# ppwwyyxx/speaker-recognition

Measured on AMD Instinct MI355X. Metric: frames/sec scored (MFCC+GMM), higher is better.
Workload: dtype f32

## Files before the change

speaker-recognition_amd/csrc/mfcc_f64.hip:

```cpp
#include "batch.hpp"
#include "mfcc.hpp"
#include "mfcc_dev.hpp"
#include "wave_ops.hpp"

#include <algorithm>

namespace sr {

static int &precision_flag() {
    static int v = 2;
    return v;
}
int mfcc_precision() { return precision_flag(); }
void mfcc_set_precision(int mode) { precision_flag() = mode == 0 ? 0 : 2; }

using d2 = double2;

__device__ __forceinline__ d2 mk(double x, double y) { return make_double2(x, y); }
__device__ __forceinline__ d2 dadd(d2 a, d2 b) { return mk(a.x + b.x, a.y + b.y); }
__device__ __forceinline__ d2 dsub(d2 a, d2 b) { return mk(a.x - b.x, a.y - b.y); }
__device__ __forceinline__ d2 dmul(d2 a, d2 b) { return mk(fma(-a.y, b.y, a.x * b.x), fma(a.y, b.x, a.x * b.y)); }
__device__ __forceinline__ d2 dmul_mi(d2 a) { return mk(a.y, -a.x); }
constexpr double DH = 0.70710678118654752440;
__device__ __forceinline__ d2 dmul_h_mh(d2 a) { return mk(DH * (a.x + a.y), DH * (a.y - a.x)); }
__device__ __forceinline__ d2 dmul_mh_mh(d2 a) { return mk(DH * (a.y - a.x), -DH * (a.x + a.y)); }

__device__ __forceinline__ d2 tw64(const d2 *t, int i, int nc) {
    d2 w = t[i & (nc - 1)];
    if (i & nc) w = mk(-w.x, -w.y);
    return w;
}

__device__ __forceinline__ void radix4d(d2 a, d2 b, d2 c, d2 d, d2 &y0, d2 &y1, d2 &y2, d2 &y3) {
    const d2 s0 = dadd(a, c), s1 = dsub(a, c), s2 = dadd(b, d), s3 = dmul_mi(dsub(b, d));
    y0 = dadd(s0, s2);
    y1 = dadd(s1, s3);
    y2 = dsub(s0, s2);
    y3 = dsub(s1, s3);
}

template <int NZ>
__device__ __forceinline__ void dft16d(d2 (&v)[16]) {
    constexpr double C1 = 0.92387953251128673848, S1 = 0.38268343236508978178;
    d2 u[4][4];
    if constexpr (NZ <= 4) {
#pragma unroll
        for (int q = 0; q < 4; q++)
#pragma unroll
            for (int r = 0; r < 4; r++) u[q][r] = v[q];
    } else {
#pragma unroll
        for (int q = 0; q < 4; q++) radix4d(v[q], v[4 + q], v[8 + q], v[12 + q], u[q][0], u[q][1], u[q][2], u[q][3]);
    }
    u[1][1] = dmul(u[1][1], mk(C1, -S1));
    u[1][2] = dmul_h_mh(u[1][2]);
    u[1][3] = dmul(u[1][3], mk(S1, -C1));
    u[2][1] = dmul_h_mh(u[2][1]);
    u[2][2] = dmul_mi(u[2][2]);
    u[2][3] = dmul_mh_mh(u[2][3]);
    u[3][1] = dmul(u[3][1], mk(S1, -C1));
    u[3][2] = dmul_mh_mh(u[3][2]);
    u[3][3] = dmul(u[3][3], mk(-C1, S1));
#pragma unroll
    for (int r = 0; r < 4; r++) radix4d(u[0][r], u[1][r], u[2][r], u[3][r], v[r], v[r + 4], v[r + 8], v[r + 12]);
}

template <int CTRL>
__device__ __forceinline__ float quad_f32(float x) {
    return __int_as_float(__builtin_amdgcn_update_dpp(0, __float_as_int(x), CTRL, 0xf, 0xf, true));
}
template <int CTRL>
__device__ __forceinline__ double quad_f64(double x) {
    union { double d; int i[2]; } a, b;
    a.d = x;
    b.i[0] = __builtin_amdgcn_update_dpp(0, a.i[0], CTRL, 0xf, 0xf, true);
    b.i[1] = __builtin_amdgcn_update_dpp(0, a.i[1], CTRL, 0xf, 0xf, true);
    return b.d;
}
constexpr int QUAD_XOR1 = 0xB1;
constexpr int QUAD_XOR2 = 0x4E;

__device__ constexpr double W32_COS[9] = {1.0, 0.98078528040323044913, 0.92387953251128675613, 0.83146961230254523708,
                                          0.70710678118654752440, 0.55557023301960222474, 0.38268343236508977173,
                                          0.19509032201612826785, 0.0};

__device__ __forceinline__ double ln_pos_f32(float e) {
    int ex;
    float m = frexpf(e, &ex);
    if (m < 0.70710678f) {
        m *= 2.0f;
        ex -= 1;
    }
    const double md = (double)m, den = md + 1.0;
    double r = (double)__builtin_amdgcn_rcpf((float)den);
    r = fma(r, fma(-den, r, 1.0), r);
    const double s = (md - 1.0) * r, s2 = s * s;
    double c15 = 1.0 / 15.0, c13 = 1.0 / 13.0, c11 = 1.0 / 11.0, c9 = 1.0 / 9.0, c7 = 1.0 / 7.0, c5 = 1.0 / 5.0, c3 = 1.0 / 3.0, ln2 = 0.69314718055994530942;
    asm volatile("" : "+s"(c15), "+s"(c13), "+s"(c11), "+s"(c9), "+s"(c7), "+s"(c5), "+s"(c3), "+s"(ln2));
    double p = c15;
    p = fma(p, s2, c13);
    p = fma(p, s2, c11);
    p = fma(p, s2, c9);
    p = fma(p, s2, c7);
    p = fma(p, s2, c5);
    p = fma(p, s2, c3);
    p = fma(p, s2, 1.0);
    return fma((double)ex, ln2, 2.0 * s * p);
}

constexpr int F64_U_ELEMS = 576;
constexpr int F64_PBUF_BYTE = F64_U_ELEMS * 16;
constexpr int F64_SE_BYTE = F64_PBUF_BYTE + 1100 * 4;
constexpr int F64_SLM_BYTE = F64_SE_BYTE + 272;
static_assert(F64_SLM_BYTE % 32 == 0 && F64_SLM_BYTE + 512 <= WAVE_SLAB_C * 16, "per-wave slab layout");

template <typename PcmT, int MP>
__global__ __launch_bounds__(64 * F64_WPB)
void mfcc_frames_fft2048_f64_kernel(const PcmT *__restrict__ pcm, const int64_t *__restrict__ sample_off,
                                    const int64_t *__restrict__ frame_off, int n_utt, int64_t n_frames,
                                    int64_t frames_per_wave, MfccDev p, MfccDev64 q, MelRuns mr, float *__restrict__ raw) {
    extern __shared__ __attribute__((aligned(32))) char smem[];
    constexpr int NC = 1024;
    float *s_melval = reinterpret_cast<float *>(smem);
    const int lane = threadIdx.x & 63;
    const int wave = threadIdx.x >> 6;
    double *s_win = reinterpret_cast<double *>(smem + (((size_t)mr.pad_floats * 4 + 31) & ~(size_t)31));
    char *slab_b = reinterpret_cast<char *>(s_win) + F64_WIN_BYTES + (size_t)wave * WAVE_SLAB_C * sizeof(d2);
    d2 *slab = reinterpret_cast<d2 *>(slab_b);
    float *pbuf = reinterpret_cast<float *>(slab_b + F64_PBUF_BYTE);
    float *s_e = reinterpret_cast<float *>(slab_b + F64_SE_BYTE);
    double *s_lm = reinterpret_cast<double *>(slab_b + F64_SLM_BYTE);

    for (int i = threadIdx.x; i < mr.pad_floats; i += 64 * F64_WPB) s_melval[i] = mr.pad_val[i];
    for (int i = threadIdx.x; i < F64_WIN_BYTES / 8; i += 64 * F64_WPB) s_win[i] = (i >= 1 && i <= p.frame_len) ? q.window[i - 1] : 0.0;
    __syncthreads();

    const d2 w1 = q.twiddle[2 * lane];
    const d2 wl = q.twiddle[lane];
    const int bb = lane & 15, gg = lane >> 4;
    const d2 w64_1 = q.twiddle[32 * bb];
    const int L = p.frame_len;
    const double lm_floor = q.mel_floor[lane];
    const int m_part = lane & 3, m_bl = lane >> 2;
    int m_c0[4];
#pragma unroll
    for (int ps = 0; ps < 4; ps++) m_c0[ps] = mr.col0[16 * ps + m_bl];

    const int64_t gwave = (int64_t)blockIdx.x * F64_WPB + wave;
    const int64_t f_begin = gwave * frames_per_wave;
    const int64_t f_end = f_begin + frames_per_wave < n_frames ? f_begin + frames_per_wave : n_frames;
    if (f_begin >= f_end) return;

    int utt = 0;
    {
        int lo = 0, hi = n_utt;
        while (hi - lo > 1) {
            const int mid = (lo + hi) >> 1;
            if (frame_off[mid] <= f_begin) lo = mid; else hi = mid;
        }
        utt = lo;
    }
    int64_t utt_f0 = frame_off[utt], utt_f1 = frame_off[utt + 1], utt_s0 = sample_off[utt];

    PcmT cm[4], c0[4], c1[4];
    auto fetch = [&](int64_t base) {
        const PcmT *fp = pcm + base;
#pragma unroll
        for (int n1 = 0; n1 < 4; n1++) {
            const int i0 = 2 * (64 * n1 + lane);
            c0[n1] = fp[min(i0, L - 1)];
            cm[n1] = fp[max(min(i0 - 1, L - 1), 0)];
            c1[n1] = fp[min(i0 + 1, L - 1)];
        }
    };
    fetch(utt_s0 + (f_begin - utt_f0) * p.frame_shift);

    for (int64_t frame = f_begin; frame < f_end; frame++) {
        d2 v[16];
#pragma unroll
        for (int n1 = 0; n1 < 4; n1++) {
            const int i0 = 2 * (64 * n1 + lane);
            const d2 wm0 = *reinterpret_cast<const d2 *>(s_win + i0);
            const double wp1 = s_win[i0 + 2];
            const double x0 = (double)c0[n1], xm = (double)cm[n1], x1 = (double)c1[n1];
            const double y0 = wm0.y * x0;
            const double re = fma(-(wm0.x * q.pre_emph), xm, y0);
            const double im = fma(-q.pre_emph, y0, wp1 * x1);
            v[n1] = mk(i0 < L ? re : 0.0, i0 + 1 < L ? im : 0.0);
        }
        if (frame + 1 < f_end) {
            int64_t nf = frame + 1;
            while (nf >= utt_f1) {
                utt++;
                utt_f0 = utt_f1;
                utt_f1 = frame_off[utt + 1];
                utt_s0 = sample_off[utt];
            }
            fetch(utt_s0 + (nf - utt_f0) * p.frame_shift);
        }
        dft16d<4>(v);
        {
            d2 cur = w1;
            v[1] = dmul(v[1], cur);
#pragma unroll
            for (int k1 = 2; k1 < 16; k1++) {
                cur = dmul(cur, w1);
                v[k1] = dmul(v[k1], cur);
            }
        }
        wave_sync();
#pragma unroll
        for (int k1 = 0; k1 < 16; k1++) slab[k1 * 68 + lane] = v[k1];
        wave_sync();
        {
            d2 w64_2 = dmul(w64_1, w64_1);
            asm volatile("" : "+v"(w64_2.x), "+v"(w64_2.y));
            const d2 w64_3 = dmul(w64_2, w64_1);
#pragma unroll
            for (int i = 0; i < 4; i++) {
                const d2 *rowp = slab + (4 * gg + i) * 68 + bb;
                radix4d(rowp[0], rowp[16], rowp[32], rowp[48], v[4 * i], v[4 * i + 1], v[4 * i + 2], v[4 * i + 3]);
                v[4 * i + 1] = dmul(v[4 * i + 1], w64_1);
                v[4 * i + 2] = dmul(v[4 * i + 2], w64_2);
                v[4 * i + 3] = dmul(v[4 * i + 3], w64_3);
            }
        }
        wave_sync();
#pragma unroll
        for (int i = 0; i < 4; i++)
#pragma unroll
            for (int c = 0; c < 4; c++) slab[((4 * gg + i) + 16 * c) * 17 + bb] = v[4 * i + c];
        wave_sync();
#pragma unroll
        for (int b = 0; b < 16; b++) v[b] = slab[lane * 17 + b];
        dft16d<16>(v);
        wave_sync();
#pragma unroll
        for (int d = 8; d < 16; d++) slab[(d - 8) * 64 + lane] = v[d];
        wave_sync();
        {
            const int src = (64 - lane) & 63;
            const int shift = lane == 0 ? 64 : 0;
#pragma unroll
            for (int d = 0; d < 8; d++) {
                const d2 zk = v[d];
                d2 zr = slab[(7 - d) * 64 + shift + src];
                if (d == 0 && lane == 0) zr = zk;
                const d2 e = mk(zk.x + zr.x, zk.y - zr.y);
                const d2 o = mk(zk.y + zr.y, zr.x - zk.x);
                d2 t;
                if (d == 0) t = dmul(wl, o);
                else if (d == 4) t = dmul(wl, dmul_h_mh(o));
                else t = dmul(wl, dmul(mk(W32_COS[d], -W32_COS[8 - d]), o));
                const d2 xp = dadd(e, t), xm = dsub(e, t);
                const int k = lane + 64 * d;
                pbuf[k] = (float)fma(xp.x, xp.x, xp.y * xp.y);
                pbuf[NC - k] = (float)fma(xm.x, xm.x, xm.y * xm.y);
            }
            if (lane == 0) pbuf[512] = (float)(4.0 * fma(v[8].x, v[8].x, v[8].y * v[8].y));
            pbuf[1025 + lane] = 0.f;
            if (lane < 11) pbuf[1089 + lane] = 0.f;
        }
        double dw[4][4];
        int dct_lane = lane;
        asm volatile("" : "+v"(dct_lane));
#pragma unroll
        for (int it = 0; it < 4; it++) {
            const double4 wv = reinterpret_cast<const double4 *>(q.dct_pad)[it * 64 + dct_lane];
            dw[it][0] = wv.x; dw[it][1] = wv.y; dw[it][2] = wv.z; dw[it][3] = wv.w;
        }
        wave_sync();
#pragma unroll
        for (int ps = 0; ps < 4; ps++) {
            const int len = mr.pass_len[ps];
            const float4 *mv4 = reinterpret_cast<const float4 *>(s_melval + mr.pass_base[ps]) + lane;
            int c0v = m_c0[ps];
            if constexpr (MP == 0) {
                int bl = 16 * ps + m_bl;
                asm volatile("" : "+v"(bl));
                c0v = mr.col0[bl];
            }
            const float4 *pp4 = reinterpret_cast<const float4 *>(pbuf + c0v) + m_part;
            float a0 = 0.f, a1 = 0.f, a2 = 0.f, a3 = 0.f;
            if constexpr (MP != 0) {
#pragma unroll
                for (int it = 0; it < mel_preset_steps(MP, ps); it++) {
                    const float4 wv = mv4[it * 64];
                    const float4 xv = pp4[it * 4];
                    a0 = fmaf(wv.x, xv.x, a0);
                    a1 = fmaf(wv.y, xv.y, a1);
                    a2 = fmaf(wv.z, xv.z, a2);
                    a3 = fmaf(wv.w, xv.w, a3);
                }
            } else {
                for (int it = 0; it < (len >> 4); it++) {
                    const float4 wv = mv4[it * 64];
                    const float4 xv = pp4[it * 4];
                    a0 = fmaf(wv.x, xv.x, a0);
                    a1 = fmaf(wv.y, xv.y, a1);
                    a2 = fmaf(wv.z, xv.z, a2);
                    a3 = fmaf(wv.w, xv.w, a3);
                }
            }
            float acc = (a0 + a1) + (a2 + a3);
            acc += quad_f32<QUAD_XOR1>(acc);
            acc += quad_f32<QUAD_XOR2>(acc);
            if (m_part == 0) s_e[16 * ps + m_bl] = acc;
        }
        wave_sync();
        {
            const float e = s_e[lane];
            s_lm[lane] = e > 0.f ? ln_pos_f32(e) : lm_floor;
        }
        wave_sync();
        {
            const int cidx = lane >> 2;
            const double4 *lp = reinterpret_cast<const double4 *>(s_lm) + m_part;
            double o0 = 0.0, o1 = 0.0;
#pragma unroll
            for (int it = 0; it < 4; it++) {
                const double4 lv = lp[it * 4];
                o0 = fma(dw[it][0], lv.x, o0);
                o1 = fma(dw[it][1], lv.y, o1);
                o0 = fma(dw[it][2], lv.z, o0);
                o1 = fma(dw[it][3], lv.w, o1);
            }
            double o = o0 + o1;
            o += quad_f64<QUAD_XOR1>(o);
            o += quad_f64<QUAD_XOR2>(o);
            if (m_part == 0 && cidx < p.n_ceps) raw[frame * p.n_ceps + cidx] = (float)o;
        }
    }
}

template <typename PcmT, int WPB>
__global__ __launch_bounds__(64 * WPB)
void mfcc_frames_f64_kernel(const PcmT *__restrict__ pcm, const int64_t *__restrict__ sample_off,
                            const int64_t *__restrict__ frame_off, int n_utt, int64_t n_frames,
                            MfccDev p, MfccDev64 q, float *__restrict__ raw ) {
    extern __shared__ __attribute__((aligned(16))) char smem[];
    const int nc = p.fft_size >> 1;
    d2 *s_tw = reinterpret_cast<d2 *>(smem);
    const int lane = threadIdx.x & 63;
    const int wave = threadIdx.x >> 6;
    d2 *buf_a = s_tw + nc + (size_t)wave * 2 * nc;
    d2 *buf_b = buf_a + nc;
    double *s_lm = reinterpret_cast<double *>(s_tw + nc + (size_t)WPB * 2 * nc) + wave * 64;

    for (int i = threadIdx.x; i < nc; i += 64 * WPB) s_tw[i] = q.twiddle[i];
    __syncthreads();

    const int64_t frames_per_iter = (int64_t)gridDim.x * WPB;
    const int64_t iters = (n_frames + frames_per_iter - 1) / frames_per_iter;
    for (int64_t it = 0; it < iters; it++) {
        const int64_t frame = (it * gridDim.x + blockIdx.x) * WPB + wave;
        const bool active = frame < n_frames;

        int64_t base = 0;
        if (active) {
            int lo = 0, hi = n_utt;
            while (hi - lo > 1) {
                const int mid = (lo + hi) >> 1;
                if (frame_off[mid] <= frame) lo = mid; else hi = mid;
            }
            base = sample_off[lo] + (frame - frame_off[lo]) * p.frame_shift;
        }

        if (active) {
            const int L = p.frame_len;
            for (int n = lane; n < nc; n += 64) {
                double re = 0.0, im = 0.0;
                const int i0 = 2 * n;
                if (i0 < L) {
                    const double c0 = (double)pcm[base + i0] * q.window[i0];
                    const double pm1 = i0 > 0 ? (double)pcm[base + i0 - 1] * q.window[i0 - 1] : 0.0;
                    re = i0 > 0 ? c0 - pm1 * q.pre_emph : c0;
                    if (i0 + 1 < L) {
                        const double c1 = (double)pcm[base + i0 + 1] * q.window[i0 + 1];
                        im = c1 - c0 * q.pre_emph;
                    }
                }
                buf_a[n] = mk(re, im);
            }
        }
        __syncthreads();

        d2 *in = buf_a, *out = buf_b;
        int ns = 1;
        for (; ns * 4 <= nc; ns *= 4) {
            if (active) {
                const int T = nc >> 2;
                const int tstep = p.fft_size / (4 * ns);
                for (int j = lane; j < T; j += 64) {
                    const int k = j & (ns - 1);
                    const int qq = k * tstep;
                    const d2 v0 = in[j];
                    const d2 v1 = dmul(in[j + T], tw64(s_tw, qq, nc));
                    const d2 v2 = dmul(in[j + 2 * T], tw64(s_tw, 2 * qq, nc));
                    const d2 v3 = dmul(in[j + 3 * T], tw64(s_tw, 3 * qq, nc));
                    d2 y0, y1, y2, y3;
                    radix4d(v0, v1, v2, v3, y0, y1, y2, y3);
                    const int j0 = ((j - k) << 2) + k;
                    out[j0] = y0;
                    out[j0 + ns] = y1;
                    out[j0 + 2 * ns] = y2;
                    out[j0 + 3 * ns] = y3;
                }
            }
            __syncthreads();
            d2 *t = in; in = out; out = t;
        }
        if (ns < nc) {
            if (active) {
                const int T = nc >> 1;
                for (int j = lane; j < T; j += 64) {
                    const d2 v0 = in[j];
                    const d2 v1 = dmul(in[j + T], tw64(s_tw, 2 * j, nc));
                    out[j] = dadd(v0, v1);
                    out[j + T] = dsub(v0, v1);
                }
            }
            __syncthreads();
            d2 *t = in; in = out; out = t;
        }

        double *pw = reinterpret_cast<double *>(out);
        if (active) {
            for (int k = lane; k <= nc; k += 64) {
                const d2 zk = in[k & (nc - 1)];
                const d2 zr = in[(nc - k) & (nc - 1)];
                const d2 e = mk(0.5 * (zk.x + zr.x), 0.5 * (zk.y - zr.y));
                const d2 o = mk(0.5 * (zk.y + zr.y), -0.5 * (zk.x - zr.x));
                const d2 x = dadd(e, dmul(tw64(s_tw, k, nc), o));
                const double pk = fma(x.x, x.x, x.y * x.y);
                pw[k] = pk < 1e-100 ? 1e-100 : pk;
            }
        }
        __syncthreads();

        if (active) {
            double mine = 0.0;
            for (int b = 0; b < p.n_filters; b++) {
                double acc = 0.0;
                const int e1 = p.mel_row[b + 1];
                for (int e = p.mel_row[b] + lane; e < e1; e += 64) acc = fma(q.mel_val[e], pw[p.mel_col[e]], acc);
                acc = wave_sum_f64(acc);
                if (lane == b) mine = acc > 0.0 ? log(acc) : q.mel_floor[b];
            }
            s_lm[lane] = mine;
        }
        __syncthreads();

        if (active && lane < p.n_ceps) {
            double acc = 0.0;
            const double *drow = q.dct + lane * p.n_filters;
            for (int b = 0; b < p.n_filters; b++) acc = fma(drow[b], s_lm[b], acc);
            raw[frame * p.n_ceps + lane] = (float)acc;
        }
        __syncthreads();
    }
}

void mfcc_launch_f64(SRMfcc &m, const MfccPlan &plan, const MfccDev &dev, int pcm_kind, const void *pcm, const int64_t *d_pcm_off,
                     const int64_t *d_raw_off, int n_utt, int64_t n_frames, float *raw) {
    auto &tabs = device_tables(m);
    const MfccDev64 dev64 = device_tables_f64(m);
    const int grid = plan.grid;
    if (plan.kernel == MFCC_F64_FAST) {
        MelRuns mr;
        mr.col0 = tabs.mel_col0.p;
        mr.pad_val = tabs.mel_pad.p;
        mr.pad_floats = tabs.mel.pad_floats;
        for (int ps = 0; ps < 4; ps++) {
            mr.pass_base[ps] = tabs.mel.pass_base[ps];
            mr.pass_len[ps] = tabs.mel.pass_len[ps];
        }
        const size_t lds_fast = plan.lds;
        const int64_t frames_per_wave = plan.frames_per_wave;
        const int preset = plan.preset;
#define SR_LAUNCH_F64(PT, MPV)                                                                              \
    do {                                                                                                     \
        auto kern = mfcc_frames_fft2048_f64_kernel<PT, MPV>;                                                 \
        SR_HIP(hipFuncSetAttribute(reinterpret_cast<const void *>(kern), hipFuncAttributeMaxDynamicSharedMemorySize, (int)lds_fast)); \
        hipLaunchKernelGGL(kern, dim3(grid), dim3(64 * F64_WPB), lds_fast, ctx().stream, static_cast<const PT *>(pcm), d_pcm_off,      \
                           d_raw_off, n_utt, n_frames, frames_per_wave, dev, dev64, mr, raw);                \
    } while (0)
#define SR_LAUNCH_F64_P(PT)                                                                                 \
    do {                                                                                                     \
        if (preset == 1) SR_LAUNCH_F64(PT, 1); else SR_LAUNCH_F64(PT, 0); \
    } while (0)
        if (pcm_kind == SRBatch::PCM16) SR_LAUNCH_F64_P(int16_t); else SR_LAUNCH_F64_P(float);
#undef SR_LAUNCH_F64_P
#undef SR_LAUNCH_F64
        return;
    }
    if (plan.kernel != MFCC_F64_GENERIC) fail("MFCC plan names no float64 kernel");
    const int wpb = plan.wpb;
    const size_t lds = plan.lds;
#define SR_LAUNCH_G64(PT, W)                                                                                \
    do {                                                                                                     \
        auto kern = mfcc_frames_f64_kernel<PT, W>;                                                           \
        SR_HIP(hipFuncSetAttribute(reinterpret_cast<const void *>(kern), hipFuncAttributeMaxDynamicSharedMemorySize, (int)lds)); \
        hipLaunchKernelGGL(kern, dim3(grid), dim3(64 * W), lds, ctx().stream, static_cast<const PT *>(pcm), d_pcm_off, d_raw_off, \
                           n_utt, n_frames, dev, dev64, raw);                                                \
    } while (0)
#define SR_LAUNCH_G64_W(PT)                                                                                 \
    do {                                                                                                     \
        if (wpb == 4) SR_LAUNCH_G64(PT, 4); else if (wpb == 2) SR_LAUNCH_G64(PT, 2); else SR_LAUNCH_G64(PT, 1); \
    } while (0)
    if (pcm_kind == SRBatch::PCM16) SR_LAUNCH_G64_W(int16_t); else SR_LAUNCH_G64_W(float);
#undef SR_LAUNCH_G64_W
#undef SR_LAUNCH_G64
}

}
```

Baseline: 35.60 million.

## Restructure f64 FFT as 8x8x8 passes with split even/odd halves and interleaved exchanges

Replaces the 16x64 decomposition of the 1024-point complex FFT with radix-8 passes (8x8x8). Samples are split into even and odd halves whose LDS exchanges are interleaved with compute through sched_group_barrier hints, and a final radix-2 combine is added. Twiddles are precomputed per lane into registers instead of chained multiplies. The mel-energy LDS round trip is removed by keeping each lane's band in a register. The change adds register pressure and many new index maps, which are checked with constexpr static_asserts.

```diff
diff --git a/speaker-recognition_amd/csrc/mfcc_f64.hip b/speaker-recognition_amd/csrc/mfcc_f64.hip
--- a/speaker-recognition_amd/csrc/mfcc_f64.hip
+++ b/speaker-recognition_amd/csrc/mfcc_f64.hip
@@ -39,30 +39,100 @@
     y3 = dsub(s1, s3);
 }
 
-template <int NZ>
-__device__ __forceinline__ void dft16d(d2 (&v)[16]) {
-    constexpr double C1 = 0.92387953251128673848, S1 = 0.38268343236508978178;
-    d2 u[4][4];
-    if constexpr (NZ <= 4) {
-#pragma unroll
-        for (int q = 0; q < 4; q++)
-#pragma unroll
-            for (int r = 0; r < 4; r++) u[q][r] = v[q];
-    } else {
-#pragma unroll
-        for (int q = 0; q < 4; q++) radix4d(v[q], v[4 + q], v[8 + q], v[12 + q], u[q][0], u[q][1], u[q][2], u[q][3]);
-    }
-    u[1][1] = dmul(u[1][1], mk(C1, -S1));
-    u[1][2] = dmul_h_mh(u[1][2]);
-    u[1][3] = dmul(u[1][3], mk(S1, -C1));
-    u[2][1] = dmul_h_mh(u[2][1]);
-    u[2][2] = dmul_mi(u[2][2]);
-    u[2][3] = dmul_mh_mh(u[2][3]);
-    u[3][1] = dmul(u[3][1], mk(S1, -C1));
-    u[3][2] = dmul_mh_mh(u[3][2]);
-    u[3][3] = dmul(u[3][3], mk(-C1, S1));
-#pragma unroll
-    for (int r = 0; r < 4; r++) radix4d(u[0][r], u[1][r], u[2][r], u[3][r], v[r], v[r + 4], v[r + 8], v[r + 12]);
+__device__ __forceinline__ void dft8d(d2 (&v)[8]) {
+    d2 e0, e1, e2, e3, o0, o1, o2, o3;
+    radix4d(v[0], v[2], v[4], v[6], e0, e1, e2, e3);
+    radix4d(v[1], v[3], v[5], v[7], o0, o1, o2, o3);
+    o1 = dmul_h_mh(o1);
+    o2 = dmul_mi(o2);
+    o3 = dmul_mh_mh(o3);
+    v[0] = dadd(e0, o0); v[4] = dsub(e0, o0);
+    v[1] = dadd(e1, o1); v[5] = dsub(e1, o1);
+    v[2] = dadd(e2, o2); v[6] = dsub(e2, o2);
+    v[3] = dadd(e3, o3); v[7] = dsub(e3, o3);
+}
+
+constexpr int F64_HALF_SLOTS = WAVE_SLAB_C / 2;
+constexpr int F64_U_ELEMS = 576;
+__host__ __device__ constexpr int f64_p2_lane(int k1, int b) { return 8 * k1 + b; }
+__host__ __device__ constexpr int f64_p3_lane(int k1, int c) { return k1 + 8 * c; }
+__host__ __device__ constexpr int f64_ex1_slot(int k1, int l) { return 64 * k1 + (l ^ (8 * (k1 & 1))); }
+__host__ __device__ constexpr int f64_ex2_slot(int k1, int b, int c) { return 8 * f64_p3_lane(k1, c) + (f64_p3_lane(k1, c) >> 1) + b; }
+__host__ __device__ constexpr int f64_bin(int lane, int reg) { return lane + 64 * reg; }
+__host__ __device__ constexpr int f64_partner_lane(int lane) { return (64 - lane) & 63; }
+__host__ __device__ constexpr int f64_partner_reg(int lane, int d) { return lane == 0 ? 16 - d : 15 - d; }
+__host__ __device__ constexpr int f64_u_slot(int lane, int reg) { return (reg - 8) * 64 + lane; }
+
+namespace f64_map_checks {
+constexpr bool lanes_bijective() {
+    bool s2[64] = {}, s3[64] = {};
+    for (int k1 = 0; k1 < 8; k1++)
+        for (int x = 0; x < 8; x++) {
+            const int l2 = f64_p2_lane(k1, x), l3 = f64_p3_lane(k1, x);
+            if (l2 < 0 || l2 >= 64 || s2[l2] || l3 < 0 || l3 >= 64 || s3[l3]) return false;
+            s2[l2] = s3[l3] = true;
+        }
+    return true;
+}
+constexpr bool ex1_injective() {
+    bool seen[512] = {};
+    for (int k1 = 0; k1 < 8; k1++)
+        for (int l = 0; l < 64; l++) {
+            const int s = f64_ex1_slot(k1, l);
+            if (s < 0 || s >= 512 || seen[s]) return false;
+            if (s != f64_ex1_slot(k1 & 1, l) - 64 * (k1 & 1) + 64 * k1) return false;
+            const int a = l >> 3, b = l & 7;
+            if (s != ((a & 1) ? f64_ex1_slot(k1, 8 + b) - 8 : f64_ex1_slot(k1, b)) + 8 * a) return false;
+            seen[s] = true;
+        }
+    return 512 <= F64_HALF_SLOTS;
+}
+constexpr bool ex2_injective() {
+    bool seen[F64_HALF_SLOTS] = {};
+    for (int k1 = 0; k1 < 8; k1++)
+        for (int b = 0; b < 8; b++)
+            for (int c = 0; c < 8; c++) {
+                const int s = f64_ex2_slot(k1, b, c);
+                if (s < 0 || s >= F64_HALF_SLOTS || seen[s]) return false;
+                if (s != f64_ex2_slot(k1, b, 0) + 68 * c) return false;
+                if (s != f64_ex2_slot(k1, 0, c) + b) return false;
+                seen[s] = true;
+            }
+    return true;
+}
+constexpr bool bins_bijective() {
+    bool seen[1024] = {};
+    for (int lane = 0; lane < 64; lane++)
+        for (int reg = 0; reg < 16; reg++) {
+            const int k = f64_bin(lane, reg);
+            if (k < 0 || k >= 1024 || seen[k]) return false;
+            seen[k] = true;
+        }
+    for (int k1 = 0; k1 < 8; k1++)
+        for (int c = 0; c < 8; c++)
+            for (int d = 0; d < 8; d++)
+                if (f64_bin(f64_p3_lane(k1, c), d) != k1 + 8 * (c + 8 * d)) return false;
+    return true;
+}
+constexpr bool partner_is_mirror() {
+    bool seen[F64_U_ELEMS] = {};
+    for (int lane = 0; lane < 64; lane++)
+        for (int reg = 8; reg < 16; reg++) {
+            const int s = f64_u_slot(lane, reg);
+            if (s < 0 || s >= 512 || seen[s]) return false;
+            seen[s] = true;
+        }
+    for (int lane = 0; lane < 64; lane++)
+        for (int d = 0; d < 8; d++) {
+            const int k = f64_bin(lane, d), pl = f64_partner_lane(lane), pr = f64_partner_reg(lane, d);
+            if (k == 0) {
+                if (f64_u_slot(pl, pr) >= F64_U_ELEMS) return false;
+                continue;
+            }
+            if (pr < 8 || pr >= 16 || f64_bin(pl, pr) != 1024 - k) return false;
+        }
+    return f64_bin(0, 8) == 512;
+}
 }
 
 template <int CTRL>
@@ -108,11 +178,16 @@
     return fma((double)ex, ln2, 2.0 * s * p);
 }
 
-constexpr int F64_U_ELEMS = 576;
 constexpr int F64_PBUF_BYTE = F64_U_ELEMS * 16;
 constexpr int F64_SE_BYTE = F64_PBUF_BYTE + 1100 * 4;
 constexpr int F64_SLM_BYTE = F64_SE_BYTE + 272;
 static_assert(F64_SLM_BYTE % 32 == 0 && F64_SLM_BYTE + 512 <= WAVE_SLAB_C * 16, "per-wave slab layout");
+static_assert(2 * F64_HALF_SLOTS <= WAVE_SLAB_C && F64_U_ELEMS <= WAVE_SLAB_C, "the two halves' exchange regions lie inside the wave's slab");
+static_assert(f64_map_checks::lanes_bijective(), "pass-2 / pass-3 lane maps are bijections onto the wave");
+static_assert(f64_map_checks::ex1_injective(), "exchange 1: (k1, lane) -> slot is a bijection onto [0, 512)");
+static_assert(f64_map_checks::ex2_injective(), "exchange 2: (k1, b, c) -> slot is injective into the half's region");
+static_assert(f64_map_checks::bins_bijective(), "(lane, register) -> bin is a bijection onto [0, 1024)");
+static_assert(f64_map_checks::partner_is_mirror(), "partner(k) is where bin 1024 - k lives");
 
 template <typename PcmT, int MP>
 __global__ __launch_bounds__(64 * F64_WPB)
@@ -128,20 +203,18 @@
     char *slab_b = reinterpret_cast<char *>(s_win) + F64_WIN_BYTES + (size_t)wave * WAVE_SLAB_C * sizeof(d2);
     d2 *slab = reinterpret_cast<d2 *>(slab_b);
     float *pbuf = reinterpret_cast<float *>(slab_b + F64_PBUF_BYTE);
-    float *s_e = reinterpret_cast<float *>(slab_b + F64_SE_BYTE);
     double *s_lm = reinterpret_cast<double *>(slab_b + F64_SLM_BYTE);
 
     for (int i = threadIdx.x; i < mr.pad_floats; i += 64 * F64_WPB) s_melval[i] = mr.pad_val[i];
     for (int i = threadIdx.x; i < F64_WIN_BYTES / 8; i += 64 * F64_WPB) s_win[i] = (i >= 1 && i <= p.frame_len) ? q.window[i - 1] : 0.0;
     __syncthreads();
 
-    const d2 w1 = q.twiddle[2 * lane];
-    const d2 wl = q.twiddle[lane];
-    const int bb = lane & 15, gg = lane >> 4;
-    const d2 w64_1 = q.twiddle[32 * bb];
+    d2 w1 = q.twiddle[2 * lane];
+    d2 wl = q.twiddle[lane];
     const int L = p.frame_len;
-    const double lm_floor = q.mel_floor[lane];
     const int m_part = lane & 3, m_bl = lane >> 2;
+    const int my_band = 16 * m_part + m_bl;
+    double lm_floor = q.mel_floor[my_band];
     int m_c0[4];
 #pragma unroll
     for (int ps = 0; ps < 4; ps++) m_c0[ps] = mr.col0[16 * ps + m_bl];
@@ -162,31 +235,83 @@
     }
     int64_t utt_f0 = frame_off[utt], utt_f1 = frame_off[utt + 1], utt_s0 = sample_off[utt];
 
-    PcmT cm[4], c0[4], c1[4];
+    d2 tw1[8], tw2[8];
+#pragma unroll
+    for (int k = 1; k < 8; k++) {
+        tw1[k] = tw64(q.twiddle, 4 * lane * k, NC);
+        tw2[k] = tw64(q.twiddle, 32 * (lane & 7) * k, NC);
+        asm volatile("" : "+v"(tw1[k].x), "+v"(tw1[k].y), "+v"(tw2[k].x), "+v"(tw2[k].y));
+    }
+    asm volatile("" : "+v"(w1.x), "+v"(w1.y), "+v"(wl.x), "+v"(wl.y), "+v"(lm_floor));
+    const int p2_k1 = lane >> 3, p2_b = lane & 7;
+    const int ex1_w_even = f64_ex1_slot(0, lane), ex1_w_odd = f64_ex1_slot(1, lane) - 64;
+    const int ex1_r_even = f64_ex1_slot(p2_k1, p2_b), ex1_r_odd = f64_ex1_slot(p2_k1, 8 + p2_b) - 8;
+    const int ex2_w = f64_ex2_slot(p2_k1, p2_b, 0);
+    const int ex2_r = f64_ex2_slot(lane & 7, 0, lane >> 3);
+    d2 *const slab_e = slab, *const slab_o = slab + F64_HALF_SLOTS;
+
+    PcmT cs[2][5];
     auto fetch = [&](int64_t base) {
         const PcmT *fp = pcm + base;
 #pragma unroll
-        for (int n1 = 0; n1 < 4; n1++) {
-            const int i0 = 2 * (64 * n1 + lane);
-            c0[n1] = fp[min(i0, L - 1)];
-            cm[n1] = fp[max(min(i0 - 1, L - 1), 0)];
-            c1[n1] = fp[min(i0 + 1, L - 1)];
+        for (int n1 = 0; n1 < 2; n1++) {
+            const int i0 = 4 * (64 * n1 + lane);
+#pragma unroll
+            for (int j = 0; j < 5; j++) cs[n1][j] = fp[max(min(i0 + j - 1, L - 1), 0)];
         }
     };
     fetch(utt_s0 + (f_begin - utt_f0) * p.frame_shift);
 
+    auto pass1 = [&](const d2 x0, const d2 x1, d2 (&v)[8]) {
+        const d2 xa = dmul_h_mh(x1), xb = dmul_mi(x1), xc = dmul_mh_mh(x1);
+        v[0] = dadd(x0, x1);
+        v[1] = dmul(dadd(x0, xa), tw1[1]);
+        v[2] = dmul(dadd(x0, xb), tw1[2]);
+        v[3] = dmul(dadd(x0, xc), tw1[3]);
+        v[4] = dmul(dsub(x0, x1), tw1[4]);
+        v[5] = dmul(dsub(x0, xa), tw1[5]);
+        v[6] = dmul(dsub(x0, xb), tw1[6]);
+        v[7] = dmul(dsub(x0, xc), tw1[7]);
+    };
+    auto ex1_write = [&](d2 *hs, const d2 (&v)[8]) {
+#pragma unroll
+        for (int k1 = 0; k1 < 8; k1++) hs[((k1 & 1) ? ex1_w_odd : ex1_w_even) + 64 * k1] = v[k1];
+    };
+    auto ex1_read = [&](const d2 *hs, d2 (&v)[8]) {
+#pragma unroll
+        for (int a = 0; a < 8; a++) v[a] = hs[((a & 1) ? ex1_r_odd : ex1_r_even) + 8 * a];
+    };
+    auto pass2 = [&](d2 (&v)[8]) {
+        dft8d(v);
+#pragma unroll
+        for (int c = 1; c < 8; c++) v[c] = dmul(v[c], tw2[c]);
+    };
+    auto ex2_write = [&](d2 *hs, const d2 (&v)[8]) {
+#pragma unroll
+        for (int c = 0; c < 8; c++) hs[ex2_w + 68 * c] = v[c];
+    };
+    auto ex2_read = [&](const d2 *hs, d2 (&v)[8]) {
+#pragma unroll
+        for (int b = 0; b < 8; b++) v[b] = hs[ex2_r + b];
+    };
+
     for (int64_t frame = f_begin; frame < f_end; frame++) {
-        d2 v[16];
-#pragma unroll
-        for (int n1 = 0; n1 < 4; n1++) {
-            const int i0 = 2 * (64 * n1 + lane);
-            const d2 wm0 = *reinterpret_cast<const d2 *>(s_win + i0);
-            const double wp1 = s_win[i0 + 2];
-            const double x0 = (double)c0[n1], xm = (double)cm[n1], x1 = (double)c1[n1];
-            const double y0 = wm0.y * x0;
-            const double re = fma(-(wm0.x * q.pre_emph), xm, y0);
-            const double im = fma(-q.pre_emph, y0, wp1 * x1);
-            v[n1] = mk(i0 < L ? re : 0.0, i0 + 1 < L ? im : 0.0);
+        d2 xe[2], xo[2];
+#pragma unroll
+        for (int n1 = 0; n1 < 2; n1++) {
+            const int i0 = 4 * (64 * n1 + lane);
+            const d2 wa = *reinterpret_cast<const d2 *>(s_win + i0);
+            const d2 wb = *reinterpret_cast<const d2 *>(s_win + i0 + 2);
+            const double wc = s_win[i0 + 4];
+            const double xm = (double)cs[n1][0], x0 = (double)cs[n1][1], x1 = (double)cs[n1][2], x2 = (double)cs[n1][3],
+                         x3 = (double)cs[n1][4];
+            const double t0 = wa.y * x0, t1 = wb.x * x1, t2 = wb.y * x2;
+            const double y0 = fma(-(wa.x * q.pre_emph), xm, t0);
+            const double y1 = fma(-q.pre_emph, t0, t1);
+            const double y2 = fma(-q.pre_emph, t1, t2);
+            const double y3 = fma(-q.pre_emph, t2, wc * x3);
+            xe[n1] = mk(i0 < L ? y0 : 0.0, i0 + 1 < L ? y1 : 0.0);
+            xo[n1] = mk(i0 + 2 < L ? y2 : 0.0, i0 + 3 < L ? y3 : 0.0);
         }
         if (frame + 1 < f_end) {
             int64_t nf = frame + 1;
@@ -198,53 +323,79 @@
             }
             fetch(utt_s0 + (nf - utt_f0) * p.frame_shift);
         }
-        dft16d<4>(v);
+        d2 ve[8], vo[8];
+#define F64_SPREAD_EXCHANGE()                                                                  \
+    do {                                                                                       \
+        _Pragma("unroll") for (int i_ = 0; i_ < 8; i_++) {                                     \
+            __builtin_amdgcn_sched_group_barrier(0x200, 1, 0);               \
+            __builtin_amdgcn_sched_group_barrier(0x002, 3, 0);           \
+        }                                                                                      \
+        _Pragma("unroll") for (int i_ = 0; i_ < 8; i_++) {                                     \
+            __builtin_amdgcn_sched_group_barrier(0x100, 1, 0);                \
+            __builtin_amdgcn_sched_group_barrier(0x002, 2, 0);                                 \
+        }                                                                                      \
+    } while (0)
+        pass1(xe[0], xe[1], ve);
+        __builtin_amdgcn_sched_barrier(0);
+        wave_sync();
+        ex1_write(slab_e, ve);
+        wave_sync();
+        ex1_read(slab_e, ve);
+        pass1(xo[0], xo[1], vo);
+        F64_SPREAD_EXCHANGE();
+        __builtin_amdgcn_sched_barrier(0);
+        ex1_write(slab_o, vo);
+        wave_sync();
+        ex1_read(slab_o, vo);
+        pass2(ve);
+        F64_SPREAD_EXCHANGE();
+        __builtin_amdgcn_sched_barrier(0);
+        wave_sync();
+        ex2_write(slab_e, ve);
+        wave_sync();
+        ex2_read(slab_e, ve);
+        pass2(vo);
+        F64_SPREAD_EXCHANGE();
+        __builtin_amdgcn_sched_barrier(0);
+        wave_sync();
+        ex2_write(slab_o, vo);
+        wave_sync();
+        ex2_read(slab_o, vo);
+        dft8d(ve);
+        F64_SPREAD_EXCHANGE();
+        __builtin_amdgcn_sched_barrier(0);
+        dft8d(vo);
+#undef F64_SPREAD_EXCHANGE
+        wave_sync();
+        d2 z512;
+#pragma unroll
+        for (int d = 0; d < 8; d++) {
+            constexpr double C1 = 0.92387953251128673848, S1 = 0.38268343236508978178;
+            d2 t = vo[d];
+            if (d == 1) t = dmul(t, mk(C1, -S1));
+            else if (d == 2) t = dmul_h_mh(t);
+            else if (d == 3) t = dmul(t, mk(S1, -C1));
+            else if (d == 4) t = dmul_mi(t);
+            else if (d == 5) t = dmul(t, mk(-S1, -C1));
+            else if (d == 6) t = dmul_mh_mh(t);
+            else if (d == 7) t = dmul(t, mk(-C1, -S1));
+            t = dmul(w1, t);
+            const d2 hi = dsub(ve[d], t);
+            ve[d] = dadd(ve[d], t);
+            slab[f64_u_slot(lane, d + 8)] = hi;
+            if (d == 0) z512 = hi;
+        }
+        wave_sync();
         {
-            d2 cur = w1;
-            v[1] = dmul(v[1], cur);
-#pragma unroll
-            for (int k1 = 2; k1 < 16; k1++) {
-                cur = dmul(cur, w1);
-                v[k1] = dmul(v[k1], cur);
-            }
-        }
-        wave_sync();
-#pragma unroll
-        for (int k1 = 0; k1 < 16; k1++) slab[k1 * 68 + lane] = v[k1];
-        wave_sync();
-        {
-            d2 w64_2 = dmul(w64_1, w64_1);
-            asm volatile("" : "+v"(w64_2.x), "+v"(w64_2.y));
-            const d2 w64_3 = dmul(w64_2, w64_1);
-#pragma unroll
-            for (int i = 0; i < 4; i++) {
-                const d2 *rowp = slab + (4 * gg + i) * 68 + bb;
-                radix4d(rowp[0], rowp[16], rowp[32], rowp[48], v[4 * i], v[4 * i + 1], v[4 * i + 2], v[4 * i + 3]);
-                v[4 * i + 1] = dmul(v[4 * i + 1], w64_1);
-                v[4 * i + 2] = dmul(v[4 * i + 2], w64_2);
-                v[4 * i + 3] = dmul(v[4 * i + 3], w64_3);
-            }
-        }
-        wave_sync();
-#pragma unroll
-        for (int i = 0; i < 4; i++)
-#pragma unroll
-            for (int c = 0; c < 4; c++) slab[((4 * gg + i) + 16 * c) * 17 + bb] = v[4 * i + c];
-        wave_sync();
-#pragma unroll
-        for (int b = 0; b < 16; b++) v[b] = slab[lane * 17 + b];
-        dft16d<16>(v);
-        wave_sync();
-#pragma unroll
-        for (int d = 8; d < 16; d++) slab[(d - 8) * 64 + lane] = v[d];
-        wave_sync();
-        {
-            const int src = (64 - lane) & 63;
-            const int shift = lane == 0 ? 64 : 0;
+            const int src = f64_partner_lane(lane);
+            d2 zp[8];
+#pragma unroll
+            for (int d = 0; d < 8; d++) zp[d] = slab[f64_u_slot(src, f64_partner_reg(lane, d))];
+            __builtin_amdgcn_sched_barrier(0);
 #pragma unroll
             for (int d = 0; d < 8; d++) {
-                const d2 zk = v[d];
-                d2 zr = slab[(7 - d) * 64 + shift + src];
+                const d2 zk = ve[d];
+                d2 zr = zp[d];
                 if (d == 0 && lane == 0) zr = zk;
                 const d2 e = mk(zk.x + zr.x, zk.y - zr.y);
                 const d2 o = mk(zk.y + zr.y, zr.x - zk.x);
@@ -253,11 +404,11 @@
                 else if (d == 4) t = dmul(wl, dmul_h_mh(o));
                 else t = dmul(wl, dmul(mk(W32_COS[d], -W32_COS[8 - d]), o));
                 const d2 xp = dadd(e, t), xm = dsub(e, t);
-                const int k = lane + 64 * d;
+                const int k = f64_bin(lane, d);
                 pbuf[k] = (float)fma(xp.x, xp.x, xp.y * xp.y);
                 pbuf[NC - k] = (float)fma(xm.x, xm.x, xm.y * xm.y);
             }
-            if (lane == 0) pbuf[512] = (float)(4.0 * fma(v[8].x, v[8].x, v[8].y * v[8].y));
+            if (lane == 0) pbuf[512] = (float)(4.0 * fma(z512.x, z512.x, z512.y * z512.y));
             pbuf[1025 + lane] = 0.f;
             if (lane < 11) pbuf[1089 + lane] = 0.f;
         }
@@ -270,6 +421,7 @@
             dw[it][0] = wv.x; dw[it][1] = wv.y; dw[it][2] = wv.z; dw[it][3] = wv.w;
         }
         wave_sync();
+        float e_band = 0.f;
 #pragma unroll
         for (int ps = 0; ps < 4; ps++) {
             const int len = mr.pass_len[ps];
@@ -305,13 +457,9 @@
             float acc = (a0 + a1) + (a2 + a3);
             acc += quad_f32<QUAD_XOR1>(acc);
             acc += quad_f32<QUAD_XOR2>(acc);
-            if (m_part == 0) s_e[16 * ps + m_bl] = acc;
-        }
-        wave_sync();
-        {
-            const float e = s_e[lane];
-            s_lm[lane] = e > 0.f ? ln_pos_f32(e) : lm_floor;
-        }
+            if (m_part == ps) e_band = acc;
+        }
+        s_lm[my_band] = e_band > 0.f ? ln_pos_f32(e_band) : lm_floor;
         wave_sync();
         {
             const int cidx = lane >> 2;
```

Result: no change. 35.80 million (median of 6 runs) (+0.6%).
